# SludgePhD/Compeg

Measured on AMD Instinct MI355X. Metric: Mpixels/s decoded (4K 4:2:2 restart-interval baseline JPEG -> RGBA8 in HBM), higher is better.
Workload: dtype u32 bit-reader / i16 levels / f32 IDCT / u8 RGBA

## Files before the change

compeg_amd/csrc/kernels.hip:

```cpp
#include <hip/hip_runtime.h>

#include <algorithm>
#include <atomic>
#include <cstdio>
#include <cstdlib>

#include "kernels_body.h"
#include "coop_body.h"
#include "walk_body.h"
#include "kernels.h"
#include "lab.h"

namespace compeg {

struct DeviceLimits {
    uint32_t cus, lds_bytes;
};
static DeviceLimits device_limits()
{
    static std::atomic<uint64_t> known[64];
    int dev = 0;
    const bool indexed = hipGetDevice(&dev) == hipSuccess && dev >= 0 && dev < 64;
    if (indexed) {
        const uint64_t k = known[dev].load(std::memory_order_relaxed);
        if (k)
            return DeviceLimits{uint32_t(k >> 32), uint32_t(k)};
    }
    int cus = 0, lds = 0;
    if (hipDeviceGetAttribute(&cus, hipDeviceAttributeMultiprocessorCount, dev) != hipSuccess || cus <= 0)
        cus = 256;
    if (hipDeviceGetAttribute(&lds, hipDeviceAttributeMaxSharedMemoryPerMultiprocessor, dev) != hipSuccess || lds < 64 * 1024)
        lds = 160 * 1024;
    if (indexed)
        known[dev].store(uint64_t(cus) << 32 | uint32_t(lds), std::memory_order_relaxed);
    if (getenv("COMPEG_VERBOSE"))
        fprintf(stderr, "[compeg] device %d: %d compute units, %d bytes of LDS each\n", dev, cus, lds);
    return DeviceLimits{uint32_t(cus), uint32_t(lds)};
}

__global__ void __launch_bounds__(1024)
huffman_kernel(const ImageDesc *__restrict__ descs, uint32_t l2_in_lds, uint32_t window_words)
{
    extern __shared__ __attribute__((aligned(16))) uint8_t smem[];
    const ImageDesc &d = descs[blockIdx.y];
    const uint32_t first_interval = blockIdx.x * blockDim.x;
    if (first_interval >= d.total_intervals)
        return;

    uint16_t *l1 = reinterpret_cast<uint16_t *>(smem);
    uint16_t *l2 = l1 + kL1Entries;
    const uint32_t wave_area = align16(window_words * 4u) + kWave * kDuSlotBytes;
    uint8_t *wave_base = smem + align16((kL1Entries + l2_in_lds) * 2u);

    stage_luts(d, l1, l2, l2_in_lds, threadIdx.x, blockDim.x);

    const uint32_t wave = threadIdx.x / kWave, lane = threadIdx.x % kWave;
    uint32_t *win = reinterpret_cast<uint32_t *>(wave_base + wave * wave_area);
    uint8_t *slots = reinterpret_cast<uint8_t *>(win) + align16(window_words * 4u);

    const uint32_t wave_first = first_interval + wave * kWave;
    uint32_t win_base = 0, win_len = 0;
    if (wave_first < d.total_intervals) {
        wave_window(d, wave_first, window_words, win_base, win_len);
        stage_window(d, win, win_base, win_len, lane);
    }
    __syncthreads();

    const uint32_t interval = wave_first + lane;
    if (interval >= d.total_intervals)
        return;

    HuffShared s;
    s.l1 = l1;
    s.l2 = l2;
    s.l2_staged = umin(l2_in_lds, d.fast_off + 2u * kFastEntries);
    s.win = win;
    s.win_base = win_base;
    s.win_len = win_len;
    s.du_slots = slots;
    huff_decode_interval(d, s, interval, lane);
}

template <bool SAMPLES>
__device__ __forceinline__ void entropy_kernel_body(const ImageDesc *__restrict__ descs, uint32_t l2_in_lds,
                                                    uint32_t window_words)
{
    extern __shared__ __attribute__((aligned(16))) uint8_t smem[];
    const ImageDesc &d = descs[blockIdx.y];
    const uint32_t first_interval = blockIdx.x * blockDim.x;
    if (first_interval >= d.total_intervals)
        return;

    uint16_t *l1 = reinterpret_cast<uint16_t *>(smem);
    uint16_t *l2 = l1 + kL1Entries;
    const uint32_t wave_area = align16(window_words * 4u) + kWave * kDuSlotBytes;
    uint8_t *wave_base = smem + align16((kL1Entries + l2_in_lds) * 2u);

    stage_luts(d, l1, l2, l2_in_lds, threadIdx.x, blockDim.x);

    const uint32_t wave = threadIdx.x / kWave, lane = threadIdx.x % kWave;
    uint32_t *win = reinterpret_cast<uint32_t *>(wave_base + wave * wave_area);
    const uint32_t wave_first = first_interval + wave * kWave;
    uint32_t win_base = 0, win_len = 0;
    if (wave_first < d.total_intervals) {
        wave_window(d, wave_first, window_words, win_base, win_len);
        stage_window(d, win, win_base, win_len, lane);
    }
    __syncthreads();

    if (wave_first >= d.total_intervals)
        return;

    HuffShared s;
    s.l1 = l1;
    s.l2 = l2;
    s.l2_staged = umin(l2_in_lds, d.fast_off + 2u * kFastEntries);
    s.win = win;
    s.win_base = win_base;
    s.win_len = win_len;
    s.du_slots = reinterpret_cast<uint8_t *>(win) + align16(window_words * 4u);
    entropy_wave_to_records<SAMPLES>(d, s, wave_first + lane, lane);
}

__global__ void __launch_bounds__(1024)
entropy_kernel(const ImageDesc *__restrict__ descs, uint32_t l2_in_lds, uint32_t window_words)
{
    entropy_kernel_body<false>(descs, l2_in_lds, window_words);
}

__global__ void __launch_bounds__(768)
entropy_samples_kernel(const ImageDesc *__restrict__ descs, uint32_t l2_in_lds, uint32_t window_words)
{
    entropy_kernel_body<true>(descs, l2_in_lds, window_words);
}

struct WindowAhead {
    const ImageDesc *descs;
    uint32_t image;
    bool any;
    uint32_t first;
    uint32_t window_words, lane;
    uint32_t *win;
    uint32_t raw_base, raw_end, base, len, sink;
    uint32_t *queue;
    uint32_t next, drawn, stride, units, waves_per_image, group;

    __device__ __forceinline__ void at(uint32_t du, uint32_t du_total)
    {
        if (queue) {
            if (du == 0u && lane == 0u)
                drawn = atomicAdd(queue, 1u);
            if (du == 1u) {
                next = (stride + uint32_t(__builtin_amdgcn_readfirstlane(int(drawn)))) * group;
                any = next < units;
                if (any) {
                    image = uint32_t(__builtin_amdgcn_readfirstlane(int(next / waves_per_image)));
                    first = uint32_t(__builtin_amdgcn_readfirstlane(int((next % waves_per_image) * kWave)));
                }
            }
        }
        if (!any)
            return;
        const ImageDesc *dn = descs + image;
        if (du == (queue ? 1u : 0u))
            wave_window_fetch(*dn, first, raw_base, raw_end);
        if (du_total >= 8u && du == (du_total >= 10u ? du_total - 8u : 2u)) {
            uint32_t b, l;
            wave_window_from(*dn, raw_base, raw_end, window_words, b, l);
            const uint32_t have = dn->nwords > b ? umin(l, dn->nwords - b) : 0u;
            auto *words = CG_GLOBAL(const uint32_t, dn->words);
            for (uint32_t v = lane * 32u; v < have; v += kWave * 32u)
                sink ^= words[b + v];
        }
        if (du_total >= 8u && du == (du_total >= 10u ? du_total - 5u : 5u))
            asm volatile("" ::"v"(sink));
    }

    __device__ __forceinline__ void decoded(uint32_t du, uint32_t du_total)
    {
        if (!any || du + 1u != du_total)
            return;
        const ImageDesc *dn = descs + image;
        uint32_t b, l;
        wave_window_from(*dn, raw_base, raw_end, window_words, b, l);
        base = uint32_t(__builtin_amdgcn_readfirstlane(int(b)));
        len = uint32_t(__builtin_amdgcn_readfirstlane(int(l)));
        stage_window(*dn, win, base, len, lane);
        __builtin_amdgcn_fence(__ATOMIC_RELEASE, "wavefront");
        __builtin_amdgcn_wave_barrier();
    }
};

template <class LAYOUT, uint32_t GROUP>
__device__ __forceinline__ void fused_kernel_body(const ImageDesc *__restrict__ descs, uint32_t l2_in_lds, uint32_t window_words,
                                                  uint32_t waves_per_image, uint32_t images, uint32_t *queue)
{
    constexpr uint32_t group = GROUP;
    extern __shared__ __attribute__((aligned(16))) uint8_t smem[];
    const uint32_t wave = uint32_t(__builtin_amdgcn_readfirstlane(int(threadIdx.x / kWave))), lane = threadIdx.x % kWave;
    uint32_t image = blockIdx.y, wave_first = (blockIdx.x * (blockDim.x / kWave) + wave) * kWave;
    bool has_work = true;
    if (waves_per_image) {
        const uint32_t flat = (blockIdx.x * (blockDim.x / kWave) + wave) * (queue ? group : 1u);
        image = flat / waves_per_image;
        wave_first = (flat % waves_per_image) * kWave;
        has_work = image < images;
        image = has_work ? image : images - 1u;
    }
    image = uint32_t(__builtin_amdgcn_readfirstlane(int(image)));
    wave_first = uint32_t(__builtin_amdgcn_readfirstlane(int(wave_first)));
    if (!waves_per_image && blockIdx.x * blockDim.x >= descs[image].total_intervals)
        return;
    has_work = has_work && wave_first < descs[image].total_intervals;

    uint16_t *l1 = reinterpret_cast<uint16_t *>(smem);
    uint16_t *l2 = l1 + kL1Entries;
    const uint32_t wave_area = align16(window_words * 4u) + kWave * kDuSlotBytes;
    uint8_t *wave_base = smem + align16((kL1Entries + l2_in_lds) * 2u);
    uint32_t *win = reinterpret_cast<uint32_t *>(wave_base + wave * wave_area);
    uint8_t *slots = reinterpret_cast<uint8_t *>(win) + align16(window_words * 4u);

    uint32_t win_base = 0, win_len = 0;
    if (has_work)
        wave_window(descs[image], wave_first, window_words, win_base, win_len);
    stage_luts_and_window(descs[image], l1, l2, l2_in_lds, threadIdx.x, blockDim.x, win, win_base, win_len, lane);
    __syncthreads();

    if (!has_work)
        return;

    const uint32_t stride = gridDim.x * (blockDim.x / kWave), units = waves_per_image * images;
    const uint32_t per_draw = waves_per_image && queue ? group : 1u;
    uint32_t flat = (blockIdx.x * (blockDim.x / kWave) + wave) * per_draw;
    for (;;) {
        const ImageDesc &d = descs[image];
        HuffShared s;
        s.l1 = l1;
        s.l2 = l2;
        s.l2_staged = umin(l2_in_lds, d.fast_off + 2u * kFastEntries);
        s.win = win;
        s.win_base = win_base;
        s.win_len = win_len;
        s.du_slots = slots;
        const bool draw = waves_per_image && queue && flat % per_draw == per_draw - 1u;
        flat += waves_per_image && queue ? 1u : stride;
        WindowAhead ahead;
        ahead.descs = descs;
        ahead.queue = draw ? queue : nullptr;
        ahead.stride = stride;
        ahead.units = units;
        ahead.waves_per_image = waves_per_image;
        ahead.group = per_draw;
        ahead.next = ahead.drawn = 0u;
        ahead.any = waves_per_image && !draw && flat < units;
        ahead.image = ahead.first = 0u;
        if (ahead.any) {
            ahead.image = uint32_t(__builtin_amdgcn_readfirstlane(int(flat / waves_per_image)));
            ahead.first = uint32_t(__builtin_amdgcn_readfirstlane(int((flat % waves_per_image) * kWave)));
        }
        ahead.window_words = window_words;
        ahead.lane = lane;
        ahead.win = win;
        ahead.sink = 0u;
        LAYOUT::decode(d, s, wave_first + lane, lane, ahead);
        if (!ahead.any)
            break;
        if (draw)
            flat = ahead.next;
        image = ahead.image;
        wave_first = ahead.first;
        win_base = ahead.base;
        win_len = ahead.len;
    }
}

constexpr uint32_t kMcuQueueGroup = 4;

template <bool WIDE, bool RECORDS = false>
struct Wave422 {
    template <class AHEAD>
    static __device__ __forceinline__ void decode(const ImageDesc &d, const HuffShared &s, uint32_t interval, uint32_t lane, AHEAD &ahead)
    {
        decode_wave_fused_422<AHEAD, WIDE, RECORDS>(d, s, interval, lane, ahead);
    }
};
#if !defined(CG_FUSED_BOUNDS) || !defined(COMPEG_LAB)
#define CG_FUSED_BOUNDS 768
#endif
__global__ void __launch_bounds__(CG_FUSED_BOUNDS)
decode_fused_422_kernel(const ImageDesc *__restrict__ descs, uint32_t l2_in_lds, uint32_t window_words,
                        uint32_t waves_per_image, uint32_t images, uint32_t *queue)
{
    fused_kernel_body<Wave422<false>, 1>(descs, l2_in_lds, window_words, waves_per_image, images, queue);
}
__global__ void __launch_bounds__(768)
decode_fused_422_mcu_kernel(const ImageDesc *__restrict__ descs, uint32_t l2_in_lds, uint32_t window_words,
                            uint32_t waves_per_image, uint32_t images, uint32_t *queue)
{
    fused_kernel_body<Wave422<true>, kMcuQueueGroup>(descs, l2_in_lds, window_words, waves_per_image, images, queue);
}
__global__ void __launch_bounds__(768)
decode_fused_422_mcu_rec_kernel(const ImageDesc *__restrict__ descs, uint32_t l2_in_lds, uint32_t window_words,
                                uint32_t waves_per_image, uint32_t images, uint32_t *queue)
{
    fused_kernel_body<Wave422<true, true>, kMcuQueueGroup>(descs, l2_in_lds, window_words, waves_per_image, images, queue);
}
template <int HS, int VS, int MC>
__device__ __forceinline__ void fused_layout_kernel_body(const ImageDesc *__restrict__ descs, uint32_t l2_in_lds, uint32_t window_words)
{
    extern __shared__ __attribute__((aligned(16))) uint8_t smem[];
    const ImageDesc &d = descs[blockIdx.y];
    const uint32_t first_interval = blockIdx.x * blockDim.x;
    if (first_interval >= d.total_intervals)
        return;
    uint16_t *l1 = reinterpret_cast<uint16_t *>(smem);
    uint16_t *l2 = l1 + kL1Entries;
    const uint32_t wave_area = align16(window_words * 4u) + kWave * kDuSlotBytes;
    uint8_t *wave_base = smem + align16((kL1Entries + l2_in_lds) * 2u);
    const uint32_t wave = uint32_t(__builtin_amdgcn_readfirstlane(int(threadIdx.x / kWave))), lane = threadIdx.x % kWave;
    uint32_t *win = reinterpret_cast<uint32_t *>(wave_base + wave * wave_area);
    const uint32_t wave_first = first_interval + wave * kWave;
    uint32_t win_base = 0, win_len = 0;
    if (wave_first < d.total_intervals)
        wave_window(d, wave_first, window_words, win_base, win_len);
    stage_luts_and_window(d, l1, l2, l2_in_lds, threadIdx.x, blockDim.x, win, win_base, win_len, lane);
    __syncthreads();
    if (wave_first >= d.total_intervals)
        return;
    HuffShared s;
    s.l1 = l1;
    s.l2 = l2;
    s.l2_staged = umin(l2_in_lds, d.fast_off + 2u * kFastEntries);
    s.win = win;
    s.win_base = win_base;
    s.win_len = win_len;
    s.du_slots = reinterpret_cast<uint8_t *>(win) + align16(window_words * 4u);
    decode_wave_fused_layout<HS, VS, MC>(d, s, wave_first + lane, lane);
}

__global__ void __launch_bounds__(512)
decode_fused_444_kernel(const ImageDesc *__restrict__ descs, uint32_t l2_in_lds, uint32_t window_words)
{
    fused_layout_kernel_body<1, 1, 2>(descs, l2_in_lds, window_words);
}
__global__ void __launch_bounds__(768)
decode_fused_444_single_kernel(const ImageDesc *__restrict__ descs, uint32_t l2_in_lds, uint32_t window_words)
{
    fused_layout_kernel_body<1, 1, 1>(descs, l2_in_lds, window_words);
}
__global__ void __launch_bounds__(512)
decode_fused_440_kernel(const ImageDesc *__restrict__ descs, uint32_t l2_in_lds, uint32_t window_words)
{
    fused_layout_kernel_body<1, 2, 2>(descs, l2_in_lds, window_words);
}
__global__ void __launch_bounds__(768)
decode_fused_440_single_kernel(const ImageDesc *__restrict__ descs, uint32_t l2_in_lds, uint32_t window_words)
{
    fused_layout_kernel_body<1, 2, 1>(descs, l2_in_lds, window_words);
}
__global__ void __launch_bounds__(512)
decode_fused_420_kernel(const ImageDesc *__restrict__ descs, uint32_t l2_in_lds, uint32_t window_words)
{
    fused_layout_kernel_body<2, 2, 1>(descs, l2_in_lds, window_words);
}

template <class WAVE>
__device__ __forceinline__ void fused_stream_kernel_body(const ImageDesc *__restrict__ descs, uint32_t l2_in_lds, uint32_t rows,
                                                         uint32_t stage_after, uint32_t stage_below, uint32_t waves_per_image, uint32_t images,
                                                         uint32_t *queue)
{
    extern __shared__ __attribute__((aligned(16))) uint8_t smem[];
    const uint32_t wave = uint32_t(__builtin_amdgcn_readfirstlane(int(threadIdx.x / kWave))), lane = threadIdx.x % kWave;
    uint32_t image = blockIdx.y, wave_first = (blockIdx.x * (blockDim.x / kWave) + wave) * kWave;
    bool has_work = true;
    if (waves_per_image) {
        const uint32_t flat = blockIdx.x * (blockDim.x / kWave) + wave;
        image = flat / waves_per_image;
        wave_first = (flat % waves_per_image) * kWave;
        has_work = image < images;
        image = has_work ? image : images - 1u;
    }
    image = uint32_t(__builtin_amdgcn_readfirstlane(int(image)));
    wave_first = uint32_t(__builtin_amdgcn_readfirstlane(int(wave_first)));
    const ImageDesc &d = descs[image];
    if (!waves_per_image && blockIdx.x * blockDim.x >= d.total_intervals)
        return;
    uint16_t *l1 = reinterpret_cast<uint16_t *>(smem);
    uint16_t *l2 = l1 + kL1Entries;
    const uint32_t wave_area = rows * kWave * 4u + kWave * kDuSlotBytes;
    uint8_t *wave_base = smem + align16((kL1Entries + l2_in_lds) * 2u);
    uint32_t *win = reinterpret_cast<uint32_t *>(wave_base + wave * wave_area);
    stage_luts_and_window(d, l1, l2, l2_in_lds, threadIdx.x, blockDim.x, win, 0u, 0u, lane);
    __syncthreads();
    if (!has_work || wave_first >= d.total_intervals)
        return;
    HuffShared s;
    s.l1 = l1;
    s.l2 = l2;
    s.l2_staged = umin(l2_in_lds, d.fast_off + 2u * kFastEntries);
    s.win = win;
    s.win_base = 0u;
    s.win_len = 0u;
    s.du_slots = reinterpret_cast<uint8_t *>(win) + rows * kWave * 4u;
    if (!waves_per_image) {
        WAVE::decode(d, s, rows, stage_after, stage_below, wave_first + lane, lane);
        return;
    }
    const uint32_t stride = gridDim.x * (blockDim.x / kWave), units = waves_per_image * images;
    for (uint32_t flat = blockIdx.x * (blockDim.x / kWave) + wave;;) {
        uint32_t drawn = 0u;
        if (queue && lane == 0u)
            drawn = atomicAdd(queue, 1u);
        WAVE::decode(descs[image], s, rows, stage_after, stage_below, wave_first + lane, lane);
        flat = queue ? stride + uint32_t(__builtin_amdgcn_readfirstlane(int(drawn))) : flat + stride;
        if (flat >= units)
            break;
        image = uint32_t(__builtin_amdgcn_readfirstlane(int(flat / waves_per_image)));
        wave_first = uint32_t(__builtin_amdgcn_readfirstlane(int((flat % waves_per_image) * kWave)));
    }
}

struct Wave422Stream {
    static __device__ __forceinline__ void decode(const ImageDesc &d, const HuffShared &s, uint32_t rows, uint32_t stage_after,
                                                  uint32_t stage_below, uint32_t interval, uint32_t lane)
    {
        decode_wave_fused_422_stream(d, s, rows, stage_after, stage_below, interval, lane);
    }
};
template <int HS, int VS, int MC>
struct WaveLayoutStream {
    static __device__ __forceinline__ void decode(const ImageDesc &d, const HuffShared &s, uint32_t rows, uint32_t stage_after,
                                                  uint32_t stage_below, uint32_t interval, uint32_t lane)
    {
        decode_wave_fused_layout<HS, VS, MC, true>(d, s, interval, lane, rows, stage_after, stage_below);
    }
};
constexpr uint32_t kWalkSpareRows = 3;
__global__ void __launch_bounds__(768)
walk_mcus_422_kernel(const ImageDesc *__restrict__ descs, uint32_t l2_in_lds, uint32_t rows, uint32_t stage_below,
                     uint32_t waves_per_image, uint32_t images, uint32_t *queue, uint32_t with_walk_tables, uint32_t chunk)
{
    extern __shared__ __attribute__((aligned(32))) uint8_t smem[];
    const uint32_t wave = uint32_t(__builtin_amdgcn_readfirstlane(int(threadIdx.x / kWave))), lane = threadIdx.x % kWave;
    uint32_t image = blockIdx.y, wave_first = (blockIdx.x * (blockDim.x / kWave) + wave) * kWave;
    bool has_work = true;
    if (waves_per_image) {
        const uint32_t flat = blockIdx.x * (blockDim.x / kWave) + wave;
        image = flat / waves_per_image;
        wave_first = (flat % waves_per_image) * kWave;
        has_work = image < images;
        image = has_work ? image : images - 1u;
    }
    image = uint32_t(__builtin_amdgcn_readfirstlane(int(image)));
    wave_first = uint32_t(__builtin_amdgcn_readfirstlane(int(wave_first)));
    const ImageDesc &d = descs[image];
    if (!waves_per_image && blockIdx.x * blockDim.x >= d.total_intervals)
        return;
    uint16_t *l1 = reinterpret_cast<uint16_t *>(smem);
    uint16_t *l2 = l1 + kL1Entries;
    const uint32_t walk_off = (align16((kL1Entries + l2_in_lds) * 2u) + 31u) & ~31u;
    uint32_t *walk = reinterpret_cast<uint32_t *>(smem + walk_off);
    const bool tables = with_walk_tables != 0u && d.walk != nullptr;
    const uint32_t dump_off = walk_off + (with_walk_tables ? kWalkWords * 4u : 0u);
    int16_t *dump = reinterpret_cast<int16_t *>(smem + dump_off);
    const uint32_t wave_area = uint32_t(kWave) * walk_list_bytes(chunk) + kWalkSlowWords * 4u + (rows + kWalkSpareRows) * kWalkRowBytes;
    uint32_t *lists = reinterpret_cast<uint32_t *>(smem + dump_off + 96u + wave * wave_area);
    uint32_t *slow_window = lists + uint32_t(kWave) * walk_list_bytes(chunk) / 4u;
    uint32_t *win = slow_window + kWalkSlowWords;
    stage_luts(d, l1, l2, l2_in_lds, threadIdx.x, blockDim.x, 2u * kDcFastEntries);
    if (tables)
        copy_words_to_lds(walk, d.walk, kWalkWords, threadIdx.x, blockDim.x);
    __syncthreads();
    if (!has_work || wave_first >= d.total_intervals)
        return;
    HuffShared s;
    s.l1 = l1;
    s.l2 = l2;
    s.l2_staged = umin(l2_in_lds, d.fast_off + 2u * kFastEntries + 2u * kDcFastEntries);
    s.win = win;
    s.win_base = 0u;
    s.win_len = 0u;
    s.du_slots = nullptr;
    WalkTabs tabs;
    walk_tabs(d, s, tables ? walk : nullptr, tabs);
    if (!waves_per_image) {
        walk_wave_422(d, s, tabs, lists, slow_window, dump, rows, stage_below, chunk, wave_first + lane, lane);
        return;
    }
    const uint32_t stride = gridDim.x * (blockDim.x / kWave), units = waves_per_image * images;
    for (uint32_t flat = blockIdx.x * (blockDim.x / kWave) + wave;;) {
        uint32_t drawn = 0u;
        if (queue && lane == 0u)
            drawn = atomicAdd(queue, 1u);
        walk_wave_422(descs[image], s, tabs, lists, slow_window, dump, rows, stage_below, chunk, wave_first + lane, lane);
        flat = queue ? stride + uint32_t(__builtin_amdgcn_readfirstlane(int(drawn))) : flat + stride;
        if (flat >= units)
            break;
        image = uint32_t(__builtin_amdgcn_readfirstlane(int(flat / waves_per_image)));
        wave_first = uint32_t(__builtin_amdgcn_readfirstlane(int((flat % waves_per_image) * kWave)));
    }
}
__global__ void __launch_bounds__(768)
decode_fused_422_stream_kernel(const ImageDesc *__restrict__ descs, uint32_t l2_in_lds, uint32_t rows, uint32_t stage_after,
                               uint32_t stage_below, uint32_t waves_per_image, uint32_t images, uint32_t *queue)
{
    fused_stream_kernel_body<Wave422Stream>(descs, l2_in_lds, rows, stage_after, stage_below, waves_per_image, images, queue);
}
__global__ void __launch_bounds__(512)
decode_fused_444_stream_kernel(const ImageDesc *__restrict__ descs, uint32_t l2_in_lds, uint32_t rows, uint32_t stage_after,
                               uint32_t stage_below, uint32_t waves_per_image, uint32_t images, uint32_t *queue)
{
    fused_stream_kernel_body<WaveLayoutStream<1, 1, 2>>(descs, l2_in_lds, rows, stage_after, stage_below, waves_per_image, images, queue);
}
__global__ void __launch_bounds__(512)
decode_fused_440_stream_kernel(const ImageDesc *__restrict__ descs, uint32_t l2_in_lds, uint32_t rows, uint32_t stage_after,
                               uint32_t stage_below, uint32_t waves_per_image, uint32_t images, uint32_t *queue)
{
    fused_stream_kernel_body<WaveLayoutStream<1, 2, 2>>(descs, l2_in_lds, rows, stage_after, stage_below, waves_per_image, images, queue);
}
__global__ void __launch_bounds__(512)
decode_fused_420_stream_kernel(const ImageDesc *__restrict__ descs, uint32_t l2_in_lds, uint32_t rows, uint32_t stage_after,
                               uint32_t stage_below, uint32_t waves_per_image, uint32_t images, uint32_t *queue)
{
    fused_stream_kernel_body<WaveLayoutStream<2, 2, 1>>(descs, l2_in_lds, rows, stage_after, stage_below, waves_per_image, images, queue);
}

__global__ void __launch_bounds__(128, 2)
decode_pair_422_kernel(const ImageDesc *__restrict__ descs, uint32_t l2_in_lds, uint32_t window_words)
{
    extern __shared__ __attribute__((aligned(16))) uint8_t smem[];
    const ImageDesc &d = descs[blockIdx.y];
    const uint32_t first_interval = blockIdx.x * kWave;
    if (first_interval >= d.total_intervals)
        return;

    uint16_t *l1 = reinterpret_cast<uint16_t *>(smem);
    uint16_t *l2 = l1 + kL1Entries;
    uint8_t *area = smem + align16((kL1Entries + l2_in_lds) * 2u);
    uint32_t *win = reinterpret_cast<uint32_t *>(area);
    uint8_t *slots = area + align16(window_words * 4u);
    int32_t *dcs = reinterpret_cast<int32_t *>(slots + 2u * kWave * kDuSlotBytes);

    const uint32_t wave = threadIdx.x / kWave, lane = threadIdx.x % kWave;
    uint32_t win_base = 0, win_len = 0;
    wave_window(d, first_interval, window_words, win_base, win_len);
    if (wave == 0)
        stage_luts_and_window(d, l1, l2, l2_in_lds, threadIdx.x, blockDim.x, win, win_base, win_len, lane);
    else
        stage_luts(d, l1, l2, l2_in_lds, threadIdx.x, blockDim.x);
    for (uint32_t i = threadIdx.x; i < 2u * kWave * kDuSlotBytes / 4u; i += blockDim.x)
        reinterpret_cast<slot_word_t *>(slots)[i] = 0u;
    __syncthreads();

    const uint32_t interval = first_interval + lane;
    const bool active = interval < d.total_intervals;
    const uint32_t du_total = d.restart_interval * 4u;

    HuffShared s;
    s.l1 = l1;
    s.l2 = l2;
    s.l2_staged = umin(l2_in_lds, d.fast_off + 2u * kFastEntries);
    s.win = win;
    s.win_base = win_base;
    s.win_len = win_len;
    s.du_slots = slots;

    if (wave == 0) {
        EntropyState e;
        if (active)
            entropy_init(e, d, s, interval);
#pragma unroll 1
        for (uint32_t du = 0; du < du_total; du++) {
            const uint32_t k = du & 3u, comp = k < 2u ? 0u : k - 1u, set = du & 1u;
            if (active) {
                uint8_t *slot = slots + (set * kWave + lane) * kDuSlotBytes;
                dcs[set * kWave + lane] = entropy_data_unit(e, d, s, comp, reinterpret_cast<int16_t *>(slot));
// ... 781 lines not shown
```

compeg_amd/csrc/kernels_body.h:

```cpp
#pragma once

#include <cstdint>
#include <cstring>

#include "device_types.h"

#if defined(__HIPCC__)
#define CG_DEV __device__ __forceinline__
#else
#define CG_DEV static inline
#endif

#if defined(__HIP_DEVICE_COMPILE__)
#define CG_GLOBAL(T, p) (reinterpret_cast<__attribute__((address_space(1))) T *>(reinterpret_cast<uintptr_t>(p)))
#define CG_PIN_SCALAR(x) asm volatile("" : "+s"(x))
#else
#define CG_GLOBAL(T, p) (p)
#define CG_PIN_SCALAR(x) (void)(x)
#endif

#ifndef CG_IDCT_PACKED
#define CG_IDCT_PACKED 1
#endif
#ifndef CG_PRIO_IDCT
#define CG_PRIO_IDCT 1
#endif
#ifndef CG_PRIO_ENTROPY
#define CG_PRIO_ENTROPY 0
#endif
#ifndef CG_PRIO_COMPOSITE
#define CG_PRIO_COMPOSITE 3
#endif
#ifndef CG_NT_STORES
#define CG_NT_STORES 1
#endif
#if !defined(COMPEG_LAB)
#undef CG_EXP
#endif
#ifndef CG_EXP
#define CG_EXP 0
#endif

namespace compeg {

struct alignas(16) Vec4u {
    uint32_t x, y, z, w;
};

template <bool STREAM>
CG_DEV void store_pixels(uint8_t *p, const Vec4u &v)
{
#if defined(COMPEG_LAB) && defined(CG_STORE_POLICY) && defined(__HIP_DEVICE_COMPILE__)
    if (STREAM) {
        typedef uint32_t u32x4 __attribute__((ext_vector_type(4)));
        const u32x4 val{v.x, v.y, v.z, v.w};
        asm volatile("global_store_dwordx4 %0, %1, off " CG_STORE_POLICY ::"v"(p), "v"(val) : "memory");
        return;
    }
#endif
#if CG_NT_STORES && defined(__HIP_DEVICE_COMPILE__)
    if (STREAM) {
        typedef uint32_t u32x4 __attribute__((ext_vector_type(4)));
        __builtin_nontemporal_store(
            u32x4{v.x, v.y, v.z, v.w},
            reinterpret_cast<__attribute__((address_space(1))) u32x4 *>(reinterpret_cast<uintptr_t>(p)));
        return;
    }
#endif
    *CG_GLOBAL(Vec4u, reinterpret_cast<Vec4u *>(p)) = v;
}


struct HuffShared {
    const uint16_t *l1;
    const uint16_t *l2;
    uint32_t l2_staged;
    const uint32_t *win;
    uint32_t win_base;
    uint32_t win_len;
    uint8_t *du_slots;
};

CG_DEV uint32_t bswap32(uint32_t w)
{
    return (w << 24) | ((w & 0xff00u) << 8) | ((w >> 8) & 0xff00u) | (w >> 24);
}

struct BitReader {
    uint32_t cur, nxt, left, next_word;
};

CG_DEV uint32_t fetch_word(const ImageDesc &d, const HuffShared &s, uint32_t idx)
{
    const uint32_t rel = idx - s.win_base;
    if (rel < s.win_len)
        return s.win[rel];
    return idx < d.nwords ? bswap32(CG_GLOBAL(const uint32_t, d.words)[idx]) : 0u;
}

CG_DEV void refill(BitReader &b, const ImageDesc &d, const HuffShared &s)
{
    if (b.left < 32u) {
        const uint32_t w = fetch_word(d, s, b.next_word);
        b.next_word += 1u;
        b.cur |= w >> (b.left & 31u);
        b.nxt = (w << 1) << ((31u - b.left) & 31u);
        b.left += 32u;
    }
}

CG_DEV void consume(BitReader &b, uint32_t n)
{
    b.cur = (b.cur << (n & 31u)) | ((b.nxt >> 1) >> ((31u - n) & 31u));
    b.nxt <<= (n & 31u);
    b.left -= n;
}

CG_DEV uint32_t peek(const BitReader &b, uint32_t n)
{
    return (b.cur >> 1) >> ((31u - n) & 31u);
}

CG_DEV int32_t huff_extend(int32_t v, uint32_t t)
{
    const int32_t vt = int32_t(1u << ((t - 1u) & 31u));
    const uint32_t ext = uint32_t(v) + (0xffffffffu << (t & 31u)) + 1u;
    return v < vt ? int32_t(ext) : v;
}

typedef uint32_t __attribute__((may_alias)) slot_word_t;
struct __attribute__((may_alias, aligned(16))) SlotVec {
    uint32_t x, y, z, w;
};

CG_DEV void zero_slot(uint8_t *slot)
{
    SlotVec *p = reinterpret_cast<SlotVec *>(slot);
#pragma unroll
    for (int i = 0; i < kRetained / 8; i++)
        p[i] = SlotVec{0u, 0u, 0u, 0u};
}

CG_DEV void take_slot(uint8_t *slot, uint32_t (&rec)[kRetained / 2])
{
    SlotVec *p = reinterpret_cast<SlotVec *>(slot);
#pragma unroll
    for (int i = 0; i < kRetained / 8; i++) {
        const SlotVec v = p[i];
        rec[4 * i + 0] = v.x;
        rec[4 * i + 1] = v.y;
        rec[4 * i + 2] = v.z;
        rec[4 * i + 3] = v.w;
    }
    zero_slot(slot);
}

constexpr uint32_t kL1Entries = 5 * 256;
constexpr uint32_t kDuWordSlack = 66;

CG_DEV uint32_t align16(uint32_t v) { return (v + 15u) & ~15u; }
CG_DEV uint32_t umin(uint32_t a, uint32_t b) { return a < b ? a : b; }
CG_DEV uint32_t umax(uint32_t a, uint32_t b) { return a > b ? a : b; }

struct __attribute__((packed, aligned(4))) Dwords4 {
    uint32_t x, y, z, w;
};

CG_DEV void copy_words_to_lds(uint32_t *dst, const uint32_t *src_, uint32_t n, uint32_t tid,
                              uint32_t nthreads)
{
    auto *src4 = CG_GLOBAL(const Dwords4, reinterpret_cast<const Dwords4 *>(src_));
    auto *src = CG_GLOBAL(const uint32_t, src_);
    const uint32_t n4 = n / 4u;
    uint32_t i = tid;
    for (; i + nthreads < n4; i += 2u * nthreads) {
        const Dwords4 a = src4[i], b = src4[i + nthreads];
        reinterpret_cast<SlotVec *>(dst)[i] = SlotVec{a.x, a.y, a.z, a.w};
        reinterpret_cast<SlotVec *>(dst)[i + nthreads] = SlotVec{b.x, b.y, b.z, b.w};
    }
    for (; i < n4; i += nthreads) {
        const Dwords4 a = src4[i];
        reinterpret_cast<SlotVec *>(dst)[i] = SlotVec{a.x, a.y, a.z, a.w};
    }
    for (uint32_t k = n4 * 4u + tid; k < n; k += nthreads)
        reinterpret_cast<slot_word_t *>(dst)[k] = src[k];
}

CG_DEV void stage_luts(const ImageDesc &d, uint16_t *l1, uint16_t *l2, uint32_t l2_in_lds,
                       uint32_t tid, uint32_t nthreads, uint32_t extra = 0u)
{
    uint32_t *dst = reinterpret_cast<uint32_t *>(l1);
    copy_words_to_lds(dst, reinterpret_cast<const uint32_t *>(d.l1), 4 * 128, tid, nthreads);
    for (uint32_t i = tid; i < 128; i += nthreads)
        reinterpret_cast<slot_word_t *>(dst)[4 * 128 + i] = 0u;
    const uint32_t n2 = umin(l2_in_lds, d.fast_off + 2u * kFastEntries + extra);
    copy_words_to_lds(reinterpret_cast<uint32_t *>(l2), reinterpret_cast<const uint32_t *>(d.l2),
                      (n2 + 1) / 2, tid, nthreads);
}

CG_DEV void wave_window_fetch(const ImageDesc &d, uint32_t wave_first, uint32_t &raw_base, uint32_t &raw_end)
{
    raw_base = wave_first < d.nstarts ? CG_GLOBAL(const uint32_t, d.starts)[wave_first] : 0u;
    const uint32_t after = wave_first + kWave;
    raw_end = (after < d.total_intervals && after < d.nstarts) ? CG_GLOBAL(const uint32_t, d.starts)[after] : d.nwords;
}

CG_DEV void wave_window_from(const ImageDesc &d, uint32_t raw_base, uint32_t raw_end, uint32_t window_words,
                             uint32_t &base, uint32_t &len)
{
    const uint32_t end = umin(raw_end, d.nwords) + kDuWordSlack + 2u;
    base = umin(raw_base, d.nwords);
    len = end > base ? umin(end - base, window_words) : 0u;
}

CG_DEV void wave_window(const ImageDesc &d, uint32_t wave_first, uint32_t window_words,
                        uint32_t &base, uint32_t &len)
{
    uint32_t raw_base, raw_end;
    wave_window_fetch(d, wave_first, raw_base, raw_end);
    wave_window_from(d, raw_base, raw_end, window_words, base, len);
}

CG_DEV SlotVec scan_words4(const ImageDesc &d, uint32_t idx)
{
    Dwords4 w{0u, 0u, 0u, 0u};
    if (idx + 3u < d.nwords) {
        w = *CG_GLOBAL(const Dwords4, reinterpret_cast<const Dwords4 *>(d.words + idx));
    } else {
        auto *words = CG_GLOBAL(const uint32_t, d.words);
        w.x = idx < d.nwords ? words[idx] : 0u;
        w.y = idx + 1u < d.nwords ? words[idx + 1u] : 0u;
        w.z = idx + 2u < d.nwords ? words[idx + 2u] : 0u;
    }
    return SlotVec{bswap32(w.x), bswap32(w.y), bswap32(w.z), bswap32(w.w)};
}

CG_DEV void window_load_round(const ImageDesc &d, uint32_t base, uint32_t len, uint32_t v0, SlotVec (&w)[8])
{
    const uint32_t nvec = (len + 3u) / 4u;
#pragma unroll
    for (int j = 0; j < 8; j++) {
        const uint32_t v = v0 + uint32_t(j) * kWave;
        w[j] = v < nvec ? scan_words4(d, base + 4u * v) : SlotVec{0u, 0u, 0u, 0u};
    }
}

CG_DEV void window_store_round(uint32_t *win, uint32_t len, uint32_t v0, const SlotVec (&w)[8])
{
    const uint32_t nvec = (len + 3u) / 4u;
    SlotVec *dst = reinterpret_cast<SlotVec *>(win);
#pragma unroll
    for (int j = 0; j < 8; j++) {
        const uint32_t v = v0 + uint32_t(j) * kWave;
        if (v < nvec)
            dst[v] = w[j];
    }
}

CG_DEV void stage_window(const ImageDesc &d, uint32_t *win, uint32_t base, uint32_t len,
                         uint32_t lane)
{
    const uint32_t nvec = (len + 3u) / 4u;
    for (uint32_t v0 = lane; v0 < nvec; v0 += 8u * kWave) {
        SlotVec w[8];
        window_load_round(d, base, len, v0, w);
        window_store_round(win, len, v0, w);
    }
}

CG_DEV void stage_luts_and_window(const ImageDesc &d, uint16_t *l1, uint16_t *l2, uint32_t l2_in_lds,
                                  uint32_t tid, uint32_t nthreads, uint32_t *win, uint32_t base, uint32_t len,
                                  uint32_t lane, uint32_t extra = 0u)
{
    SlotVec w[8];
    window_load_round(d, base, len, lane, w);
    stage_luts(d, l1, l2, l2_in_lds, tid, nthreads, extra);
    window_store_round(win, len, lane, w);
    const uint32_t nvec = (len + 3u) / 4u;
    for (uint32_t v0 = lane + 8u * kWave; v0 < nvec; v0 += 8u * kWave) {
        window_load_round(d, base, len, v0, w);
        window_store_round(win, len, v0, w);
    }
}

CG_DEV void huff_decode_interval(const ImageDesc &d, const HuffShared &s, uint32_t interval,
                                 uint32_t lane)
{
    uint8_t *slot = s.du_slots + lane * kDuSlotBytes;
    int16_t *slot16 = reinterpret_cast<int16_t *>(slot);
    zero_slot(slot);

    BitReader b;
    b.next_word = interval < d.nstarts ? CG_GLOBAL(const uint32_t, d.starts)[interval] : 0u;
    b.cur = b.nxt = b.left = 0u;
    refill(b, d, s);

    int32_t pred0 = 0, pred1 = 0, pred2 = 0;
    const uint32_t dpm = d.dus_per_mcu;
    const uint32_t du_count = d.restart_interval * dpm;
    uint32_t du_global = interval * du_count;
    uint32_t du_local = 0;
    uint32_t k = 0;
    uint32_t comp = d.comp_of_du & 3u;
    uint32_t dc_off = d.dc_table[0] * 256u, ac_off = d.ac_table[0] * 256u;
    if (comp == 1u) {
        dc_off = d.dc_table[1] * 256u;
        ac_off = d.ac_table[1] * 256u;
    } else if (comp == 2u) {
        dc_off = d.dc_table[2] * 256u;
        ac_off = d.ac_table[2] * 256u;
    }
    uint32_t pos = 0;

    while (du_local < du_count) {
        const bool is_dc = pos == 0u;
        if (!is_dc || d.standard_entropy)
            refill(b, d, s);

        const uint32_t code = b.cur >> 16;
        uint32_t e = s.l1[(is_dc ? dc_off : ac_off) + (code >> 8)];
        if (e & 0x8000u) {
            const uint32_t idx = (e & 0x7fffu) + (code & 0xffu);
            e = idx >= d.l2_entries ? 0u : (idx < s.l2_staged ? s.l2[idx] : CG_GLOBAL(const uint16_t, d.l2)[idx]);
        }
        consume(b, e >> 8);
        const uint32_t sym = e & 0xffu;

        const uint32_t nbits = is_dc ? sym : (sym & 15u);
        const int32_t raw = int32_t(peek(b, nbits));
        consume(b, nbits);
        const int32_t val = huff_extend(raw, nbits);

        bool du_done = false;
        if (is_dc) {
            int32_t p = comp == 0u ? pred0 : (comp == 1u ? pred1 : pred2);
            p = int32_t(uint32_t(p) + uint32_t(val));
            if (comp == 0u)
                pred0 = p;
            else if (comp == 1u)
                pred1 = p;
            else
                pred2 = p;
            const uint32_t q0 = comp == 0u ? d.dc_quant[0] : (comp == 1u ? d.dc_quant[1] : d.dc_quant[2]);
            CG_GLOBAL(int32_t, d.dc)[du_global] = int32_t(uint32_t(p) * q0);
            pos = 1u;
        } else if (sym == 0u) {
            du_done = true;
        } else {
            const uint32_t p = pos + (sym >> 4);
            const bool zrl = sym == 0xf0u;
            if (!zrl && p < uint32_t(kRetained))
                slot16[p] = int16_t(val);
            pos = p + ((zrl && !d.standard_entropy) ? 2u : 1u);
            du_done = pos >= 64u;
        }

        if (du_done) {
            uint32_t rec[kRetained / 2];
            take_slot(slot, rec);
            auto *dst = CG_GLOBAL(Vec4u, reinterpret_cast<Vec4u *>(d.ac + size_t(du_global) * kRetained));
#pragma unroll
            for (int i = 0; i < 4; i++)
                dst[i] = Vec4u{rec[4 * i], rec[4 * i + 1], rec[4 * i + 2], rec[4 * i + 3]};

            du_local++;
            du_global++;
            pos = 0u;
            k = k + 1u == dpm ? 0u : k + 1u;
            comp = (d.comp_of_du >> (2u * k)) & 3u;
            dc_off = (comp == 0u ? d.dc_table[0] : (comp == 1u ? d.dc_table[1] : d.dc_table[2])) * 256u;
            ac_off = (comp == 0u ? d.ac_table[0] : (comp == 1u ? d.ac_table[1] : d.ac_table[2])) * 256u;
        }
    }
}


#define CG_S0 ((float)1.0)
#define CG_S1 ((float)1.387039845)
#define CG_S2 ((float)1.306562965)
#define CG_S3 ((float)1.175875602)
#define CG_S4 ((float)1.0)
#define CG_S5 ((float)0.785694958)
#define CG_S6 ((float)0.541196100)
#define CG_S7 ((float)0.275899379)
#define CG_C1414 ((float)1.414213562)
#define CG_C1847 ((float)1.847759065)
#define CG_C1082 ((float)1.082392200)
#define CG_C2613 ((float)2.613125930)

CG_DEV float aan_scale(int i)
{
    switch (i) {
    case 0: return CG_S0;
    case 1: return CG_S1;
    case 2: return CG_S2;
    case 3: return CG_S3;
    case 4: return CG_S4;
    case 5: return CG_S5;
    case 6: return CG_S6;
    default: return CG_S7;
    }
}

CG_DEV int zigzag_of(int natural)
{
    constexpr int8_t t[64] = {0,  1,  5,  6,  14, 15, 27, 28, 2,  4,  7,  13, 16, 26, 29, 42,
                              3,  8,  12, 17, 25, 30, 41, 43, 9,  11, 18, 24, 31, 40, 44, 53,
                              10, 19, 23, 32, 39, 45, 52, 54, 20, 22, 33, 38, 46, 51, 55, 60,
                              21, 34, 37, 47, 50, 56, 59, 61, 35, 36, 48, 49, 57, 58, 62, 63};
    return t[natural];
}

#if defined(__clang__)
typedef float f32x2 __attribute__((ext_vector_type(2)));
#else
typedef float f32x2 __attribute__((vector_size(8)));
#endif
CG_DEV float aan_splat(float c, float) { return c; }
CG_DEV f32x2 aan_splat(float c, f32x2) { return f32x2{c, c}; }
template <class T> CG_DEV T aan_const(float c)
{
    return aan_splat(c, T{});
}

template <class T, int STRIDE, bool ROW_PASS>
CG_DEV void aan_core(const T *v, T (&e)[4], T (&o)[4])
{
    T in0 = v[0 * STRIDE];
    const T in1 = v[1 * STRIDE], in2 = v[2 * STRIDE], in3 = v[3 * STRIDE];
    const T in4 = v[4 * STRIDE], in5 = v[5 * STRIDE], in6 = v[6 * STRIDE], in7 = v[7 * STRIDE];
    if (ROW_PASS)
        in0 = in0 + aan_const<T>(128.5f);
    const T tmp10 = in0 + in4, tmp11 = in0 - in4;
    const T tmp13 = in2 + in6;
    const T tmp12 = (in2 - in6) * aan_const<T>(CG_C1414) - tmp13;
    e[0] = tmp10 + tmp13;
    e[3] = tmp10 - tmp13;
    e[1] = tmp11 + tmp12;
    e[2] = tmp11 - tmp12;
    const T z13 = in5 + in3, z10 = in5 - in3;
    const T z11 = in1 + in7, z12 = in1 - in7;
    const T o7 = z11 + z13;
    const T t11 = (z11 - z13) * aan_const<T>(CG_C1414);
    const T z5 = (z10 + z12) * aan_const<T>(CG_C1847);
    const T t10 = z5 - z12 * aan_const<T>(CG_C1082);
    const T t12 = z5 - z10 * aan_const<T>(CG_C2613);
    const T o6 = t12 - o7;
    const T o5 = t11 - o6;
    const T o4 = t10 - o5;
    o[0] = o7;
    o[1] = o6;
    o[2] = o5;
    o[3] = o4;
}

template <class T, int STRIDE, bool ROW_PASS>
CG_DEV void aan_1d(T *v)
{
    T e[4], o[4];
    aan_core<T, STRIDE, ROW_PASS>(v, e, o);
#pragma unroll
    for (int k = 0; k < 4; k++) {
        v[k * STRIDE] = e[k] + o[k];
        v[(7 - k) * STRIDE] = e[k] - o[k];
    }
}

template <int HALF>
CG_DEV f32x2 aan_cross(f32x2 e, f32x2 o)
{
#if defined(__HIP_DEVICE_COMPILE__)
    f32x2 r;
    if (HALF == 0)
        asm("v_pk_add_f32 %0, %1, %2 op_sel:[0,0] op_sel_hi:[0,0] neg_hi:[0,1]" : "=v"(r) : "v"(e), "v"(o));
    else
        asm("v_pk_add_f32 %0, %1, %2 op_sel:[1,1] op_sel_hi:[1,1] neg_hi:[0,1]" : "=v"(r) : "v"(e), "v"(o));
    return r;
#else
    return f32x2{e[HALF] + o[HALF], e[HALF] - o[HALF]};
#endif
}

CG_DEV uint32_t sample_u8(float f)
{
    float m = f > 0.0f ? f : 0.0f;
    m = m < 255.0f ? m : 255.0f;
    return uint32_t(m);
}

CG_DEV void pack_rows3(const float *f0, const float *f1, const float *f2, uint32_t *o)
{
#if defined(__HIP_DEVICE_COMPILE__)
    asm volatile("s_setreg_imm32_b32 hwreg(HW_REG_MODE, 0, 2), 3\n\t"
                 "v_cvt_pk_u8_f32 %0, %6, 0, 0\n\t"
                 "v_cvt_pk_u8_f32 %0, %7, 1, %0\n\t"
                 "v_cvt_pk_u8_f32 %0, %8, 2, %0\n\t"
                 "v_cvt_pk_u8_f32 %0, %9, 3, %0\n\t"
                 "v_cvt_pk_u8_f32 %1, %10, 0, 0\n\t"
                 "v_cvt_pk_u8_f32 %1, %11, 1, %1\n\t"
                 "v_cvt_pk_u8_f32 %1, %12, 2, %1\n\t"
                 "v_cvt_pk_u8_f32 %1, %13, 3, %1\n\t"
                 "v_cvt_pk_u8_f32 %2, %14, 0, 0\n\t"
                 "v_cvt_pk_u8_f32 %2, %15, 1, %2\n\t"
                 "v_cvt_pk_u8_f32 %2, %16, 2, %2\n\t"
                 "v_cvt_pk_u8_f32 %2, %17, 3, %2\n\t"
                 "v_cvt_pk_u8_f32 %3, %18, 0, 0\n\t"
                 "v_cvt_pk_u8_f32 %3, %19, 1, %3\n\t"
                 "v_cvt_pk_u8_f32 %3, %20, 2, %3\n\t"
                 "v_cvt_pk_u8_f32 %3, %21, 3, %3\n\t"
                 "v_cvt_pk_u8_f32 %4, %22, 0, 0\n\t"
                 "v_cvt_pk_u8_f32 %4, %23, 1, %4\n\t"
                 "v_cvt_pk_u8_f32 %4, %24, 2, %4\n\t"
                 "v_cvt_pk_u8_f32 %4, %25, 3, %4\n\t"
                 "v_cvt_pk_u8_f32 %5, %26, 0, 0\n\t"
                 "v_cvt_pk_u8_f32 %5, %27, 1, %5\n\t"
                 "v_cvt_pk_u8_f32 %5, %28, 2, %5\n\t"
                 "v_cvt_pk_u8_f32 %5, %29, 3, %5\n\t"
                 "s_setreg_imm32_b32 hwreg(HW_REG_MODE, 0, 2), 0"
                 : "=&v"(o[0]), "=&v"(o[1]), "=&v"(o[2]), "=&v"(o[3]), "=&v"(o[4]), "=&v"(o[5])
                 : "v"(f0[0]), "v"(f0[1]), "v"(f0[2]), "v"(f0[3]), "v"(f0[4]), "v"(f0[5]), "v"(f0[6]), "v"(f0[7]), "v"(f1[0]), "v"(f1[1]), "v"(f1[2]), "v"(f1[3]), "v"(f1[4]), "v"(f1[5]), "v"(f1[6]), "v"(f1[7]), "v"(f2[0]), "v"(f2[1]), "v"(f2[2]), "v"(f2[3]), "v"(f2[4]), "v"(f2[5]), "v"(f2[6]), "v"(f2[7]));
#else
    o[0] = sample_u8(f0[0]) | sample_u8(f0[1]) << 8 | sample_u8(f0[2]) << 16 | sample_u8(f0[3]) << 24;
    o[1] = sample_u8(f0[4]) | sample_u8(f0[5]) << 8 | sample_u8(f0[6]) << 16 | sample_u8(f0[7]) << 24;
    o[2] = sample_u8(f1[0]) | sample_u8(f1[1]) << 8 | sample_u8(f1[2]) << 16 | sample_u8(f1[3]) << 24;
    o[3] = sample_u8(f1[4]) | sample_u8(f1[5]) << 8 | sample_u8(f1[6]) << 16 | sample_u8(f1[7]) << 24;
    o[4] = sample_u8(f2[0]) | sample_u8(f2[1]) << 8 | sample_u8(f2[2]) << 16 | sample_u8(f2[3]) << 24;
    o[5] = sample_u8(f2[4]) | sample_u8(f2[5]) << 8 | sample_u8(f2[6]) << 16 | sample_u8(f2[7]) << 24;
#endif
}

CG_DEV void pack_rows2(const float *f0, const float *f1, uint32_t *o)
{
#if defined(__HIP_DEVICE_COMPILE__)
    asm volatile("s_setreg_imm32_b32 hwreg(HW_REG_MODE, 0, 2), 3\n\t"
                 "v_cvt_pk_u8_f32 %0, %4, 0, 0\n\t"
                 "v_cvt_pk_u8_f32 %0, %5, 1, %0\n\t"
                 "v_cvt_pk_u8_f32 %0, %6, 2, %0\n\t"
                 "v_cvt_pk_u8_f32 %0, %7, 3, %0\n\t"
                 "v_cvt_pk_u8_f32 %1, %8, 0, 0\n\t"
                 "v_cvt_pk_u8_f32 %1, %9, 1, %1\n\t"
                 "v_cvt_pk_u8_f32 %1, %10, 2, %1\n\t"
                 "v_cvt_pk_u8_f32 %1, %11, 3, %1\n\t"
                 "v_cvt_pk_u8_f32 %2, %12, 0, 0\n\t"
                 "v_cvt_pk_u8_f32 %2, %13, 1, %2\n\t"
                 "v_cvt_pk_u8_f32 %2, %14, 2, %2\n\t"
                 "v_cvt_pk_u8_f32 %2, %15, 3, %2\n\t"
                 "v_cvt_pk_u8_f32 %3, %16, 0, 0\n\t"
                 "v_cvt_pk_u8_f32 %3, %17, 1, %3\n\t"
                 "v_cvt_pk_u8_f32 %3, %18, 2, %3\n\t"
                 "v_cvt_pk_u8_f32 %3, %19, 3, %3\n\t"
                 "s_setreg_imm32_b32 hwreg(HW_REG_MODE, 0, 2), 0"
                 : "=&v"(o[0]), "=&v"(o[1]), "=&v"(o[2]), "=&v"(o[3])
                 : "v"(f0[0]), "v"(f0[1]), "v"(f0[2]), "v"(f0[3]), "v"(f0[4]), "v"(f0[5]), "v"(f0[6]), "v"(f0[7]), "v"(f1[0]), "v"(f1[1]), "v"(f1[2]), "v"(f1[3]), "v"(f1[4]), "v"(f1[5]), "v"(f1[6]), "v"(f1[7]));
#else
    o[0] = sample_u8(f0[0]) | sample_u8(f0[1]) << 8 | sample_u8(f0[2]) << 16 | sample_u8(f0[3]) << 24;
    o[1] = sample_u8(f0[4]) | sample_u8(f0[5]) << 8 | sample_u8(f0[6]) << 16 | sample_u8(f0[7]) << 24;
    o[2] = sample_u8(f1[0]) | sample_u8(f1[1]) << 8 | sample_u8(f1[2]) << 16 | sample_u8(f1[3]) << 24;
    o[3] = sample_u8(f1[4]) | sample_u8(f1[5]) << 8 | sample_u8(f1[6]) << 16 | sample_u8(f1[7]) << 24;
// ... 1681 lines not shown
```

Baseline: 780,500.

## Restructure wave work-queue lookahead and window staging in fused decode

Reworks how the fused kernel's wave prefetches its next unit. The atomic queue draw moves from the start of decode to the end, and it now reserves one group further ahead (2*stride). The next unit's window bounds are read through scalar (constant address space) loads, and the L2 warm-up touch is collapsed into a single step at du 0. Staging of the next window now splits batched 16-byte loads into two halves so the loads issue together. It also adds an experimental CG_EXP==19 path without lookahead. The aim is to cut the atomic latency and the per-DU bookkeeping during decode. The trade-offs are that the queue latency is now exposed at the end of the unit, and that queue ordering and scheduling semantics change.

Result: no change. 785,200 (median of 4 runs) (+0.6%).

```diff
diff --git a/compeg_amd/csrc/kernels.hip b/compeg_amd/csrc/kernels.hip
--- a/compeg_amd/csrc/kernels.hip
+++ b/compeg_amd/csrc/kernels.hip
@@ -141,39 +141,22 @@
     uint32_t first;
     uint32_t window_words, lane;
     uint32_t *win;
-    uint32_t raw_base, raw_end, base, len, sink;
+    uint32_t base, len, sink;
     uint32_t *queue;
-    uint32_t next, drawn, stride, units, waves_per_image, group;
+    uint32_t after, stride, group;
 
     __device__ __forceinline__ void at(uint32_t du, uint32_t du_total)
     {
-        if (queue) {
-            if (du == 0u && lane == 0u)
-                drawn = atomicAdd(queue, 1u);
-            if (du == 1u) {
-                next = (stride + uint32_t(__builtin_amdgcn_readfirstlane(int(drawn)))) * group;
-                any = next < units;
-                if (any) {
-                    image = uint32_t(__builtin_amdgcn_readfirstlane(int(next / waves_per_image)));
-                    first = uint32_t(__builtin_amdgcn_readfirstlane(int((next % waves_per_image) * kWave)));
-                }
-            }
-        }
-        if (!any)
+        if (!any || du != 0u || du_total < 8u)
             return;
         const ImageDesc *dn = descs + image;
-        if (du == (queue ? 1u : 0u))
-            wave_window_fetch(*dn, first, raw_base, raw_end);
-        if (du_total >= 8u && du == (du_total >= 10u ? du_total - 8u : 2u)) {
-            uint32_t b, l;
-            wave_window_from(*dn, raw_base, raw_end, window_words, b, l);
-            const uint32_t have = dn->nwords > b ? umin(l, dn->nwords - b) : 0u;
-            auto *words = CG_GLOBAL(const uint32_t, dn->words);
-            for (uint32_t v = lane * 32u; v < have; v += kWave * 32u)
-                sink ^= words[b + v];
-        }
-        if (du_total >= 8u && du == (du_total >= 10u ? du_total - 5u : 5u))
-            asm volatile("" ::"v"(sink));
+        uint32_t raw_base, raw_end, b, l;
+        wave_window_fetch_uniform(*dn, first, raw_base, raw_end);
+        wave_window_from(*dn, raw_base, raw_end, window_words, b, l);
+        const uint32_t have = dn->nwords > b ? umin(l, dn->nwords - b) : 0u;
+        auto *words = CG_GLOBAL(const uint32_t, dn->words);
+        for (uint32_t v = lane * 32u; v < have; v += kWave * 32u)
+            sink ^= words[b + v];
     }
 
     __device__ __forceinline__ void decoded(uint32_t du, uint32_t du_total)
@@ -181,11 +164,19 @@
         if (!any || du + 1u != du_total)
             return;
         const ImageDesc *dn = descs + image;
-        uint32_t b, l;
-        wave_window_from(*dn, raw_base, raw_end, window_words, b, l);
-        base = uint32_t(__builtin_amdgcn_readfirstlane(int(b)));
-        len = uint32_t(__builtin_amdgcn_readfirstlane(int(l)));
-        stage_window(*dn, win, base, len, lane);
+        uint32_t raw_base, raw_end, drawn = 0u;
+        if (queue && lane == 0u) {
+            uint32_t zero = 0u;
+            asm volatile("" : "+v"(zero));
+            drawn = atomicAdd(queue + zero, 1u);
+        }
+        wave_window_fetch_uniform(*dn, first, raw_base, raw_end);
+        wave_window_from(*dn, raw_base, raw_end, window_words, base, len);
+        stage_window_together(*dn, win, base, len, lane);
+        asm volatile("" : "+v"(drawn)::"memory");
+        if (queue)
+            after = (2u * stride + uint32_t(__builtin_amdgcn_readfirstlane(int(drawn)))) * group;
+        asm volatile("" ::"v"(sink));
         __builtin_amdgcn_fence(__ATOMIC_RELEASE, "wavefront");
         __builtin_amdgcn_wave_barrier();
     }
@@ -231,7 +222,28 @@
 
     const uint32_t stride = gridDim.x * (blockDim.x / kWave), units = waves_per_image * images;
     const uint32_t per_draw = waves_per_image && queue ? group : 1u;
-    uint32_t flat = (blockIdx.x * (blockDim.x / kWave) + wave) * per_draw;
+    const uint32_t place = blockIdx.x * (blockDim.x / kWave) + wave;
+#if CG_EXP == 19
+    const ImageDesc &d = descs[image];
+    HuffShared s;
+    s.l1 = l1;
+    s.l2 = l2;
+    s.l2_staged = umin(l2_in_lds, d.fast_off + 2u * kFastEntries);
+    s.win = win;
+    s.win_base = win_base;
+    s.win_len = win_len;
+    s.du_slots = slots;
+    uint32_t u = place * per_draw;
+#pragma unroll 1
+    do {
+        NothingAhead none;
+        LAYOUT::decode(d, s, wave_first + lane, lane, none);
+        __builtin_amdgcn_wave_barrier();
+        u = (u + 1u) % per_draw ? u + 1u : u + 1u + (stride - 1u) * per_draw;
+    } while (waves_per_image && u < units);
+#else
+    uint32_t flat = place * per_draw;
+    uint32_t next_group = (place + stride) * per_draw;
     for (;;) {
         const ImageDesc &d = descs[image];
         HuffShared s;
@@ -242,36 +254,37 @@
         s.win_base = win_base;
         s.win_len = win_len;
         s.du_slots = slots;
-        const bool draw = waves_per_image && queue && flat % per_draw == per_draw - 1u;
-        flat += waves_per_image && queue ? 1u : stride;
+        const bool group_ends = flat % per_draw == per_draw - 1u;
+        const uint32_t next = group_ends ? next_group : flat + 1u;
         WindowAhead ahead;
         ahead.descs = descs;
-        ahead.queue = draw ? queue : nullptr;
+        ahead.any = waves_per_image && next < units;
+        ahead.queue = group_ends && ahead.any ? queue : nullptr;
         ahead.stride = stride;
-        ahead.units = units;
-        ahead.waves_per_image = waves_per_image;
         ahead.group = per_draw;
-        ahead.next = ahead.drawn = 0u;
-        ahead.any = waves_per_image && !draw && flat < units;
+        ahead.after = 0u;
         ahead.image = ahead.first = 0u;
         if (ahead.any) {
-            ahead.image = uint32_t(__builtin_amdgcn_readfirstlane(int(flat / waves_per_image)));
-            ahead.first = uint32_t(__builtin_amdgcn_readfirstlane(int((flat % waves_per_image) * kWave)));
+            ahead.image = uint32_t(__builtin_amdgcn_readfirstlane(int(next / waves_per_image)));
+            ahead.first = uint32_t(__builtin_amdgcn_readfirstlane(int((next % waves_per_image) * kWave)));
         }
         ahead.window_words = window_words;
         ahead.lane = lane;
         ahead.win = win;
         ahead.sink = 0u;
+        ahead.base = ahead.len = 0u;
         LAYOUT::decode(d, s, wave_first + lane, lane, ahead);
         if (!ahead.any)
             break;
-        if (draw)
-            flat = ahead.next;
+        flat = ahead.image * waves_per_image + ahead.first / kWave;
+        if (group_ends)
+            next_group = ahead.queue ? ahead.after : next_group + stride * per_draw;
         image = ahead.image;
         wave_first = ahead.first;
         win_base = ahead.base;
         win_len = ahead.len;
     }
+#endif
 }
 
 constexpr uint32_t kMcuQueueGroup = 4;
diff --git a/compeg_amd/csrc/kernels_body.h b/compeg_amd/csrc/kernels_body.h
--- a/compeg_amd/csrc/kernels_body.h
+++ b/compeg_amd/csrc/kernels_body.h
@@ -14,8 +14,10 @@
 #if defined(__HIP_DEVICE_COMPILE__)
 #define CG_GLOBAL(T, p) (reinterpret_cast<__attribute__((address_space(1))) T *>(reinterpret_cast<uintptr_t>(p)))
 #define CG_PIN_SCALAR(x) asm volatile("" : "+s"(x))
+#define CG_UNIFORM(T, p) (reinterpret_cast<__attribute__((address_space(4))) T *>(reinterpret_cast<uintptr_t>(p)))
 #else
 #define CG_GLOBAL(T, p) (p)
+#define CG_UNIFORM(T, p) (p)
 #define CG_PIN_SCALAR(x) (void)(x)
 #endif
 
@@ -205,6 +207,13 @@
     raw_end = (after < d.total_intervals && after < d.nstarts) ? CG_GLOBAL(const uint32_t, d.starts)[after] : d.nwords;
 }
 
+CG_DEV void wave_window_fetch_uniform(const ImageDesc &d, uint32_t wave_first, uint32_t &raw_base, uint32_t &raw_end)
+{
+    raw_base = wave_first < d.nstarts ? CG_UNIFORM(const uint32_t, d.starts)[wave_first] : 0u;
+    const uint32_t after = wave_first + kWave;
+    raw_end = (after < d.total_intervals && after < d.nstarts) ? CG_UNIFORM(const uint32_t, d.starts)[after] : d.nwords;
+}
+
 CG_DEV void wave_window_from(const ImageDesc &d, uint32_t raw_base, uint32_t raw_end, uint32_t window_words,
                              uint32_t &base, uint32_t &len)
 {
@@ -254,6 +263,58 @@
         const uint32_t v = v0 + uint32_t(j) * kWave;
         if (v < nvec)
             dst[v] = w[j];
+    }
+}
+
+template <int J0, int J1>
+CG_DEV void window_load_together(const ImageDesc &d, uint32_t base, uint32_t len, uint32_t v0, SlotVec (&w)[8])
+{
+    const uint32_t nvec = (len + 3u) / 4u;
+    auto *words = CG_GLOBAL(const uint32_t, d.words);
+    Dwords4 q[8];
+    if (d.nwords >= 4u) {
+#pragma unroll
+        for (int j = J0; j < J1; j++) {
+            const uint32_t v = v0 + uint32_t(j) * kWave, idx = base + 4u * v;
+            const bool whole = v < nvec && idx + 3u < d.nwords;
+            q[j] = *CG_GLOBAL(const Dwords4, reinterpret_cast<const Dwords4 *>(d.words + (whole ? idx : 0u)));
+        }
+    }
+#pragma unroll
+    for (int j = J0; j < J1; j++) {
+        const uint32_t v = v0 + uint32_t(j) * kWave, idx = base + 4u * v;
+        const bool whole = d.nwords >= 4u && v < nvec && idx + 3u < d.nwords;
+        w[j] = whole ? SlotVec{bswap32(q[j].x), bswap32(q[j].y), bswap32(q[j].z), bswap32(q[j].w)} : SlotVec{0u, 0u, 0u, 0u};
+        if (v < nvec && !whole) {
+            w[j].x = idx < d.nwords ? bswap32(words[idx]) : 0u;
+            w[j].y = idx + 1u < d.nwords ? bswap32(words[idx + 1u]) : 0u;
+            w[j].z = idx + 2u < d.nwords ? bswap32(words[idx + 2u]) : 0u;
+        }
+    }
+}
+
+template <int J0, int J1>
+CG_DEV void window_store_part(uint32_t *win, uint32_t len, uint32_t v0, const SlotVec (&w)[8])
+{
+    const uint32_t nvec = (len + 3u) / 4u;
+    SlotVec *dst = reinterpret_cast<SlotVec *>(win);
+#pragma unroll
+    for (int j = J0; j < J1; j++) {
+        const uint32_t v = v0 + uint32_t(j) * kWave;
+        if (v < nvec)
+            dst[v] = w[j];
+    }
+}
+
+CG_DEV void stage_window_together(const ImageDesc &d, uint32_t *win, uint32_t base, uint32_t len, uint32_t lane)
+{
+    const uint32_t nvec = (len + 3u) / 4u;
+    for (uint32_t v0 = lane; v0 < nvec; v0 += 8u * kWave) {
+        SlotVec w[8];
+        window_load_together<0, 4>(d, base, len, v0, w);
+        window_store_part<0, 4>(win, len, v0, w);
+        window_load_together<4, 8>(d, base, len, v0, w);
+        window_store_part<4, 8>(win, len, v0, w);
     }
 }
 
```
